# auggiemarignier/pxmcmc

Measured on AMD Instinct MI355X. Metric: MYULA samples/sec at L=256 synthesis, higher is better.
Workload: dtype f64

## Files before the change

### include/pxmcmc_amd.h

```cpp
#ifndef PXMCMC_AMD_H
#define PXMCMC_AMD_H

#include <stddef.h>
#include <stdint.h>

#ifdef __cplusplus
extern "C" {
#endif

typedef struct pxm_sht_plan_s* pxm_sht_plan_t;
typedef struct pxm_wav_plan_s* pxm_wav_plan_t;
typedef struct pxm_dwav_plan_s* pxm_dwav_plan_t;
typedef struct pxm_hwav_plan_s* pxm_hwav_plan_t;
typedef void* pxm_stream_t;

int pxm_version(void);
#ifdef PXM_NOISE_F64
#error "the -DPXM_NOISE_F64 build switch was removed: pass the flag PXM_NOISE_F64 per call (one library serves both precisions)"
#endif
#define PXM_NOISE_F64 16
int pxm_noise_bits(void);
int64_t pxm_host_check_address_ranges(int L, double B, int J_min, int spin, int max_chains, int what);
const char* pxm_last_error(void);
int pxm_device_count(void);
// ... 74 lines not shown

#define PXM_MODE_REAL_NOISE 0
#define PXM_MODE_CPLX_NOISE 1
#define PXM_MODE_REAL_PAIRS 2
int pxm_wav_gradg_step(pxm_wav_plan_t plan, const void* X, const void* preds, const void* data,
                       const void* invcov, int invcov_complex, const double* T, double T_scalar,
                       double delta, double lmda, const void* noise, int mode,
                       uint64_t seed, uint64_t chain0, uint64_t iter, void* X_out, int C,
                       pxm_stream_t stream);

int pxm_wav_image_init(pxm_wav_plan_t plan, const void* preds, const void* data, const void* invcov,
                       int invcov_complex, int C, pxm_stream_t stream);
int pxm_wav_image_step(pxm_wav_plan_t plan, const void* X, const void* data, const void* invcov,
                       int invcov_complex, const double* T, double T_scalar, double delta, double lmda,
                       const void* noise, int mode, uint64_t seed, uint64_t chain0, uint64_t iter,
                       void* X_out, void* preds_out, int C, pxm_stream_t stream);

int pxm_wav_ring_set_data(pxm_wav_plan_t plan, const void* data, pxm_stream_t stream);
int pxm_wav_ring_init(pxm_wav_plan_t plan, const void* X, int C, pxm_stream_t stream);
int pxm_wav_ring_step(pxm_wav_plan_t plan, const void* X, double w_re, double w_im, const double* T,
                      double T_scalar, double delta, double lmda, const void* noise, int mode,
                      uint64_t seed, uint64_t chain0, uint64_t iter, void* X_out, int C, pxm_stream_t stream);
int pxm_wav_ring_preds(pxm_wav_plan_t plan, void* preds, int C, pxm_stream_t stream);

int pxm_wav_wl_attach(pxm_wav_plan_t plan, const int32_t* pix2data, const double* weight, int64_t ndata);
int pxm_wav_wl_uses_recursion(pxm_wav_plan_t plan);
int pxm_wav_wl_forward(pxm_wav_plan_t plan, const void* X, void* gamma, int C, pxm_stream_t stream);
int pxm_wav_wl_adjoint(pxm_wav_plan_t plan, const void* gamma, const void* data, const void* invcov,
                       int invcov_complex, void* X_out, int C, pxm_stream_t stream);

int pxm_soft(const void* X, const double* T, double T_scalar, void* out, int64_t n, int C, int dtype,
             pxm_stream_t stream);
int pxm_residual_grad(const void* preds, const void* data, const void* invcov, int invcov_complex,
                      void* out, int64_t n, int C, int dtype, pxm_stream_t stream);
int pxm_myula_step(const void* X, const void* gradg, const double* T, double T_scalar,
                   const double* delta_dev, double delta, double lmda, const void* noise,
                   int noise_complex, uint64_t seed, uint64_t chain0, uint64_t iter,
                   const uint64_t* iter_dev, void* X_out, int64_t n, int C, int dtype,
                   pxm_stream_t stream);
int pxm_chain_step(const void* X, const void* proxf, const void* gradg, const double* delta_dev,
                   double delta, double lmda, const void* noise, int noise_complex, uint64_t seed,
                   uint64_t chain0, uint64_t iter, const uint64_t* iter_dev, void* X_out, int64_t n,
                   int C, int dtype, pxm_stream_t stream);
int pxm_skrock_stage(const void* U, const void* proxf, const double* T, double T_scalar, const void* gradg,
                     const void* V, double a, double b, double c, double e, double r, const void* noise,
                     int noise_complex, uint64_t seed, uint64_t chain0, uint64_t iter, const uint64_t* iter_dev,
// ... 53 lines not shown
```

### pxmcmc_amd/_lib.py

```python
import ctypes as C
import os

import torch

_HERE = os.path.dirname(os.path.abspath(__file__))
LIB_PATH = os.environ.get("PXM_LIB_PATH") or os.path.join(_HERE, "lib", "libpxmcmc_amd.so")

c_i64, c_u64, c_int, c_dbl, c_vp = C.c_int64, C.c_uint64, C.c_int, C.c_double, C.c_void_p

SIGNATURES = {
    "pxm_version": (c_int, []),
    "pxm_noise_bits": (c_int, []),
    "pxm_host_check_address_ranges": (c_i64, [c_int, c_dbl, c_int, c_int, c_int, c_int]),
    "pxm_last_error": (C.c_char_p, []),
    "pxm_device_count": (c_int, []),
    "pxm_capture_begin": (c_int, []),
    "pxm_capture_end": (c_int, []),
    "pxm_deferred_pending": (c_int, []),
    "pxm_tables_trim": (c_int, []),
    "pxm_wav_set_iter_counter": (c_int, [c_vp, c_vp]),
    "pxm_wav_release_iter_counter": (c_int, [c_vp, c_vp]),
    "pxm_wav_iter_counter_add": (c_int, [c_vp, c_u64, c_vp]),
    "pxm_wav_exact_dft_scales": (c_int, [c_vp]),
    "pxm_wav_status": (c_int, [c_vp, c_int, c_vp]),
    "pxm_sht_status": (c_int, [c_vp, c_int, c_vp]),
    "pxm_wav_profile_enable": (c_int, [c_vp, c_int]),
    "pxm_wav_profile_read": (c_int, [c_vp, c_vp, c_vp, c_vp, c_vp]),
    "pxm_wav_profile_read_launches": (c_int, [c_vp, c_vp, c_vp, c_vp, c_i64, c_vp]),
    "pxm_wav_profile_read_dft": (c_int, [c_vp, c_vp, c_vp, c_vp]),
    "pxm_wav_workspace_nonfinite": (c_i64, [c_vp, c_vp]),
    "pxm_reduce_scratch_doubles": (c_i64, [c_int]),
    "pxm_j_max": (c_int, [c_int, c_dbl]),
    "pxm_wav_bandlimits": (c_int, [c_int, c_dbl, c_int, c_vp, c_int]),
    "pxm_wav_ncoefs": (c_i64, [c_int, c_dbl, c_int, c_vp]),
    "pxm_tiling_axisym": (c_int, [c_int, c_dbl, c_int, c_vp, c_vp]),
    "pxm_mw_ring_weights": (c_int, [c_int, c_vp]),
# ... 146 lines not shown
```

### pxmcmc_amd/csrc/plans.hip

```cpp
#include "../../include/pxmcmc_amd.h"
#include "elem.h"
#include "sht_core.h"
#include "sht_rec.h"

#include <algorithm>
#include <cmath>
#include <cstdlib>
#include <cstring>
#include <map>
#include <string>
#include <memory>
#include <mutex>

namespace pxm {

struct TaskList {
  GemmTask* d = nullptr;
  int n = 0;
  bool paired = false;
  int nslab = 2;
  std::vector<int> bls;
  std::vector<int> los;
  double mfma_units = 0;
  bool gram = false;
  double gram_table_bytes = 0;
  int flags = 0;
  int pk = 0;
  std::vector<char> tab_shared;
};

static int upload_tasks(std::vector<GemmTask> v, bool paired, TaskList* out, std::vector<int> bls, int ncol,
                        const double* ws_base, const char* name, std::vector<int> los = {}, int pk = 0,
                        std::vector<char> tab_shared = {}) {
  out->pk = pk;
  tab_shared.resize(bls.size(), 0);
  out->tab_shared = tab_shared;
  out->bls = bls;
  los.resize(bls.size(), 0);
  out->los = los;
  const char* order_env = getenv("PXM_GEMM_ORDER");
  const std::string order = order_env ? order_env : (v.size() > 2048 ? "xcd" : "bins");
  const int64_t fixed = order == "xcd" ? 32 : 0;
  auto work = [fixed](const GemmTask& a) { return (int64_t)(a.k_end - a.k_beg + fixed) * a.n_rt; };
  std::stable_sort(v.begin(), v.end(), [&](const GemmTask& a, const GemmTask& b) { return work(a) > work(b); });
  if (order == "xcd" && !v.empty()) {
    constexpr int NQ = 8;
    std::map<int64_t, int> unit_of;
    std::vector<std::vector<GemmTask>> units;
    for (const GemmTask& t : v) {
      auto it = unit_of.find(t.x_off[0]);
// ... 57 lines not shown
    }
    v.swap(ordered);
  }
  out->n = (int)v.size();
  out->paired = paired;
  out->nslab = pk ? 4 : (paired ? 2 : 1);
  for (const GemmTask& t : v) {
    PXM_REQUIRE(t.n_rt >= 0 && t.n_rt <= 8 && t.row0 >= 0 && t.row0 % 16 == 0 && t.k_beg >= 0 && t.k_beg % 16 == 0 &&
                    (t.n_rt == 0 || (t.k_end > t.k_beg && (t.k_end - t.k_beg) % 16 == 0)),
                "upload_tasks: malformed GEMM task");
    out->mfma_units += (double)t.n_rt * ((t.k_end - t.k_beg) / 4) * (pk ? 1 : t.nslab);
    for (int sl = 0; sl < 4; ++sl)
      if (t.x2_off[sl]) out->flags |= 1;
    if (t.ks_off[0] || t.ks_off[1]) out->flags |= 2;
  }
  if (v.empty()) return 0;
  if (int rc = check_gemm_task_ranges(v, out->nslab, out->flags, ncol, ws_base, name)) return rc;
  if (int rc = dev_alloc(&out->d, v.size() * sizeof(GemmTask), "GEMM task list")) return rc;
  return dev_upload(out->d, v.data(), v.size() * sizeof(GemmTask));
}

static double tasklist_bytes(const TaskList& tl, int cg) {
  double bytes = 0;
  for (size_t i = 0; i < tl.bls.size(); ++i) {
    const double Ld = tl.bls[i];
    if (tl.gram) bytes += tl.gram_table_bytes + 3 * 16.0 * cg * Ld * Ld + 16.0 * Ld * Ld;
    else bytes += gemm_alg_bytes(tl.bls[i], tl.paired, cg, tl.los[i]);
    if (!tl.gram && tl.pk && tl.tab_shared[i]) bytes -= gemm_table_bytes(tl.bls[i], tl.paired, tl.los[i]);
  }
  return bytes;
}

static int run_tasks(const TaskList& tl, const double* X, double* Y, int ncol, int C, hipStream_t st,
                     const GemmAffine& aff = GemmAffine(), Profiler* prof = nullptr) {
  note_stream(st);
  if (tl.pk)
    return launch_gemm_packed(tl.d, tl.n, tl.pk, tl.flags, X, Y, ncol, 0, tasklist_bytes(tl, C), tl.mfma_units * 2048.0, st, prof);
  for (int col0 = 0; col0 < ncol; col0 += 32) {
    const int ct = (ncol - col0 >= 32) ? 2 : 1;
    const int cg = std::max(0, std::min(C - col0 / 2, 8 * ct));
    if (cg == 0) break;
    const double bytes = tasklist_bytes(tl, cg);
    GemmAffine a = aff;
    if (col0) a.bump = nullptr;
    a.ncol_live = 2 * C;
    int rc = launch_gemm(tl.d, tl.n, tl.nslab, tl.flags, X, Y, ncol, col0, ct, bytes, tl.mfma_units * ct * 2048.0, st, a, prof);
// ... 213 lines not shown
  *out = &sp;
  return 0;
}
}

struct pxm_wav_plan_s {
  int L = 0, J_min = 0, J_max = 0, Cmax = 0, Cp = 0, ncol = 0, Rp = 0;
  int spin = 0;
  double B = 0;
  int nsc = 0;
  std::vector<int> bl;
  std::vector<int64_t> coef_off;
  int64_t ncoefs = 0;
  std::vector<ShtTables*> T;
  ShtTables* TL = nullptr;
  std::vector<DftPlan> dft;
  DftPlan dftL;
  double* ws = nullptr;
  std::vector<int64_t> offG;
  int64_t offGL = 0, offHL = 0, offS = 0;
  int64_t offGD = 0, offHD = 0;
  int64_t offHDc = 0;
  TaskList gram, adj_invadj_D;
  bool have_data_rings = false;
  int64_t offHA = 0, offHB = 0;
  double* d_kc_syn = nullptr;
  double* d_kc_ana = nullptr;
  TaskList syn_fwd, syn_inv, adj_invadj, adj_fwdadj;
  TaskList ana_fwd, ana_inv, anadj_invadj, anadj_fwdadj;
  int64_t table_bytes[2] = {0, 0};
  static constexpr int NSIDE = 3;
  static constexpr int nside = 2;
  hipStream_t side[NSIDE] = {nullptr, nullptr, nullptr};
  hipEvent_t ev_fork = nullptr, ev_join[NSIDE] = {nullptr, nullptr, nullptr};
  bool plain_group = true;
  std::vector<int> lane_of;
  DftGroupList dft_group;
  int pk = 0;
  int twin_s = -1;
  bool wl_failed = false;
  double* d_twin = nullptr;
  int64_t offGT = 0;
  int ncol_t = 0;
  double* d_g2n = nullptr;
  int ncol_g2 = 0;
  double* d_hn = nullptr;
// ... 136 lines not shown
    wav_hold(p, p->T[s]);
    rc = make_dft_plan(p->bl[s], &p->dft[s]);
    if (rc) return rc;
    p->dft[s].d_status = p->d_status;
  }
  rc = get_tables(L, spin, 0xF, &p->TL);
  if (rc) return rc;
  wav_hold(p, p->TL);
  rc = make_dft_plan(L, &p->dftL);
  if (rc) return rc;
  p->dftL.d_status = p->d_status;
  int64_t w = 0;
  p->offGL = w; w += arr_size(L, p->ncol);
  p->offHL = w; w += arr_size(L, p->ncol);
  p->offGD = w; w += arr_size(L, p->ncol);
  p->offHD = w; w += arr_size(L, p->ncol);
  p->offHDc = w; w += (int64_t)(2 * L - 1) * p->Rp * 2;
  p->offHA = w; w += arr_size(L, p->ncol);
  p->offHB = w; w += arr_size(L, p->ncol);
  p->plain_group = !getenv("PXM_NO_PLAIN_DFT_GROUP");
  for (int s = 0; s < p->nsc; ++s) {
    p->offG.push_back(w); w += arr_size(p->bl[s], p->ncol);
  }
  p->offG2 = w; w += arr_size(L, p->ncol);
  p->offS = w; w += (int64_t)p->Rp * p->ncol;
  if ((rc = dev_alloc(&p->ws, (size_t)w * sizeof(double), "wavelet plan workspace"))) return rc;
  if ((rc = dev_zero(p->ws, (size_t)w * sizeof(double)))) return rc;
  std::vector<double> k0, kap;
  tiling_axisym(L, B, J_min, k0, kap);
  std::vector<double> kc_syn((size_t)p->nsc * p->Rp, 0.0), kc_ana((size_t)p->nsc * p->Rp, 0.0);
  const double cs = std::sqrt(2.0 * M_PI), ca = 1.0 / std::sqrt(2.0 * M_PI);
  for (int s = 0; s < p->nsc; ++s)
    for (int el = std::abs(spin); el < p->bl[s]; ++el) {
      const double k = (s == 0) ? k0[el] : kap[(size_t)(J_min + s - 1) * L + el];
      kc_syn[(size_t)s * p->Rp + el] = (s == 0) ? k : cs * k;
      kc_ana[(size_t)s * p->Rp + el] = (s == 0) ? k : ca * k;
    }
  if ((rc = dev_alloc(&p->d_kc_syn, kc_syn.size() * sizeof(double), "synthesis kernel rows c kappa [nsc][Rp]"))) return rc;
  if ((rc = dev_alloc(&p->d_kc_ana, kc_ana.size() * sizeof(double), "analysis kernel rows c kappa [nsc][Rp]"))) return rc;
  if ((rc = dev_upload(p->d_kc_syn, kc_syn.data(), kc_syn.size() * sizeof(double)))) return rc;
  if ((rc = dev_upload(p->d_kc_ana, kc_ana.data(), kc_ana.size() * sizeof(double)))) return rc;
  std::vector<int> el_lo(p->nsc, 0);
  for (int s = 0; s < p->nsc; ++s)
    while (el_lo[s] < p->bl[s] && kc_syn[(size_t)s * p->Rp + el_lo[s]] == 0.0) ++el_lo[s];
  std::vector<GemmTask> v_syn_fwd, v_adj_fwdadj, v_ana_inv, v_anadj_invadj, v;
  p->el_lo_s = el_lo;
// ... 60 lines not shown

extern "C" {

int pxm_wav_plan_create(int L, double B, int J_min, int max_chains, unsigned flags, pxm_wav_plan_t* plan) {
  (void)flags;
  return wav_plan_create_impl("pxm_wav_plan_create", L, B, J_min, 0, max_chains, plan);
}

int pxm_wav_plan_create_spin(int L, double B, int J_min, int spin, int max_chains, unsigned flags, pxm_wav_plan_t* plan) {
  (void)flags;
  return wav_plan_create_impl("pxm_wav_plan_create_spin", L, B, J_min, spin, max_chains, plan);
}

int pxm_wav_plan_destroy(pxm_wav_plan_t p) {
  if (!p) return 0;
  dft_group_destroy(&p->dft_group);
  for (auto& d : p->dft) free_dft_plan(&d);
  free_dft_plan(&p->dftL);
  deferred_free(p->ws);
  deferred_free(p->d_kc_syn);
  deferred_free(p->d_kc_ana);
  deferred_free(p->d_wlk);
  deferred_free(p->d_status);
  TaskList* tls[] = {&p->syn_fwd, &p->syn_inv, &p->adj_invadj, &p->adj_fwdadj, &p->gram, &p->adj_invadj_D,
                     &p->ana_fwd, &p->ana_inv, &p->anadj_invadj, &p->anadj_fwdadj, &p->wl_inv, &p->wl_invadj};
  for (TaskList* t : tls) free_tasks(t);
  profiler_release(&p->prof);
  for (ShtTables* T : p->held) release_tables(T);
  rec_tables_destroy(p->rec2);
  deferred_free(p->d_twin);
  deferred_free(p->d_g2n);
  deferred_free(p->d_hn);
  deferred_free(p->d_gn);
  dft_group_destroy(&p->dft_group_n);
  free_tasks(&p->wl_syn_fwd);
  free_tasks(&p->wl_adj_fwdadj);
  delete p;
  drain_deferred();
  return 0;
}

int pxm_wav_set_iter_counter(pxm_wav_plan_t p, uint64_t* counter_dev) {
  PXM_REQUIRE(p, "pxm_wav_set_iter_counter: null plan");
  PXM_REQUIRE(!counter_dev || !p->iter_dev || p->iter_dev == counter_dev,
              "pxm_wav_set_iter_counter: this plan already has a live iteration counter (one stepping engine per plan "
              "at a time; release the first with pxm_wav_release_iter_counter)");
  p->iter_dev = counter_dev;
// ... 329 lines not shown
    if ((rc = wav_rings_update_rings(p, out, C, st))) return rc;
  } else {
    if ((rc = wav_rings_to_blocks(p, out, C, st))) return rc;
    if ((rc = wav_blocks_to_rings(p, X_out, C, st))) return rc;
  }
  if ((rc = run_tasks(p->syn_fwd, p->ws, p->ws, p->ncol, C, st, GemmAffine(), &p->prof))) return rc;
  if ((rc = run_tasks(p->syn_inv, p->ws, p->ws, p->ncol, C, st, GemmAffine(), &p->prof))) return rc;
  PxOut po;
  po.f = (double*)preds_out;
  po.chain_stride = (int64_t)p->L * (2 * p->L - 1);
  if (dft_can_fuse(p->dftL)) {
    image_residual(po, data, invcov, invcov_complex);
    return launch_ring2px2ring(p->dftL, p->ws + p->offGL, p->ncol, po, C, st);
  }
  if ((rc = launch_ring2px(p->dftL, p->ws + p->offGL, p->ncol, po, C, st))) return rc;
  return pxm_wav_image_init(p, preds_out, data, invcov, invcov_complex, C, stream);
}

}
namespace pxm {
__global__ void k_pack_data_term(const double2* __restrict__ HD, double2* __restrict__ HDc, int64_t rows, int Cp) {
  for (int64_t i = blockIdx.x * (int64_t)blockDim.x + threadIdx.x; i < rows; i += (int64_t)gridDim.x * blockDim.x) HDc[i] = HD[i * Cp];
}
}
extern "C" {

static int wav_make_gram_lists(pxm_wav_plan_t p) {
  int rc;
  if (!p->gram.d) {
    if ((rc = get_tables(p->L, p->spin, 1u << TAB_GRAM, &p->TL))) return rc;
    wav_hold(p, p->TL);
    std::vector<GemmTask> v;
    GemmFuse fz;
    fz.x2_base = p->offHB;
    fz.hd_base = p->offHDc;
    fz.hd_stride = 2;
    append_gemm_tasks(*p->TL, TAB_GRAM, p->ncol, p->offHA, p->L, p->Rp, p->offHL, p->L, p->Rp, nullptr, p->offS, p->ws, v, 0, fz);
    if ((rc = upload_tasks(v, p->TL->paired, &p->gram, {p->L}, p->ncol, p->ws, "Gram step"))) return rc;
    p->gram.gram = true;
    p->gram.gram_table_bytes = (double)p->TL->bytes[TAB_GRAM];
    v.clear();
    append_gemm_tasks(*p->TL, TAB_INV_ADJ, p->ncol, p->offGD, p->L, p->Rp, p->offHD, p->L, p->Rp, nullptr, p->offS, p->ws, v);
    if ((rc = upload_tasks(v, p->TL->paired, &p->adj_invadj_D, {p->L}, p->ncol, p->ws, "inverse-adjoint of the data rings"))) return rc;
  }
  return 0;
}

int pxm_wav_ring_set_data(pxm_wav_plan_t p, const void* data, pxm_stream_t stream) {
  PXM_REQUIRE(p && data, "pxm_wav_ring_set_data: null argument");
  hipStream_t st = (hipStream_t)stream;
  int rc;
  if ((rc = wav_make_gram_lists(p))) return rc;
  PxIn in;
  in.f = (const double*)data;
  in.chain_stride = (int64_t)p->L * (2 * p->L - 1);
  if ((rc = launch_px2ring(p->dftL, in, p->ws + p->offGD, p->ncol, 1, st))) return rc;
  if ((rc = run_tasks(p->adj_invadj_D, p->ws, p->ws, p->ncol, 1, st, GemmAffine(), &p->prof))) return rc;
  const int64_t rows = (int64_t)(2 * p->L - 1) * p->Rp;
  hipLaunchKernelGGL(k_pack_data_term, dim3((unsigned)std::min<int64_t>((rows + 255) / 256, 2048)), dim3(256), 0, st,
                     reinterpret_cast<const double2*>(p->ws + p->offHD), reinterpret_cast<double2*>(p->ws + p->offHDc), rows,
                     p->ncol / 2);
  PXM_HIP(hipGetLastError());
  p->have_data_rings = true;
  return 0;
}

static int wav_coeffs_to_rings(pxm_wav_plan_t p, const void* X, int C, hipStream_t st, uint64_t* bump = nullptr) {
  int rc;
  if ((rc = wav_blocks_to_rings(p, X, C, st, bump))) return rc;
  return run_tasks(p->syn_fwd, p->ws, p->ws, p->ncol, C, st, GemmAffine(), &p->prof);
}

int pxm_wav_ring_init(pxm_wav_plan_t p, const void* X, int C, pxm_stream_t stream) {
  int rc = wav_check(p, X, X, C, "pxm_wav_ring_init");
  return rc ? rc : wav_coeffs_to_rings(p, X, C, (hipStream_t)stream);
}

int pxm_wav_ring_preds(pxm_wav_plan_t p, void* preds, int C, pxm_stream_t stream) {
  int rc = wav_check(p, preds, preds, C, "pxm_wav_ring_preds");
// ... 1 lines not shown
  hipStream_t st = (hipStream_t)stream;
  if ((rc = run_tasks(p->syn_inv, p->ws, p->ws, p->ncol, C, st, GemmAffine(), &p->prof))) return rc;
  PxOut out;
  out.f = (double*)preds;
  out.chain_stride = (int64_t)p->L * (2 * p->L - 1);
  return launch_ring2px(p->dftL, p->ws + p->offGL, p->ncol, out, C, st);
}

int pxm_wav_ring_step(pxm_wav_plan_t p, const void* X, double w_re, double w_im, const double* T, double T_scalar,
                      double delta, double lmda, const void* noise, int mode, uint64_t seed, uint64_t chain0,
                      uint64_t iter, void* X_out, int C, pxm_stream_t stream) {
  int rc = wav_check(p, X, X_out, C, "pxm_wav_ring_step");
  if (rc) return rc;
  PXM_REQUIRE(p->have_data_rings, "pxm_wav_ring_step: call pxm_wav_ring_set_data first");
  PxOut out;
  if ((rc = wav_update_out(p, "pxm_wav_ring_step", X, T, T_scalar, delta, lmda, noise, mode, seed, chain0, iter, X_out, &out))) return rc;
  hipStream_t st = (hipStream_t)stream;
  GemmAffine aff;
  aff.on = 1;
  aff.ns = (double)(2 * p->L - 1);
  aff.wr = w_re;
  aff.wi = w_im;
  aff.bump = p->iter_dev;
  if ((rc = run_tasks(p->gram, p->ws, p->ws, p->ncol, C, st, aff, &p->prof))) return rc;
  if ((rc = run_tasks(p->adj_fwdadj, p->ws, p->ws, p->ncol, C, st, GemmAffine(), &p->prof))) return rc;
  if (wav_can_fuse_dft(p)) {
    if ((rc = wav_rings_update_rings(p, out, C, st))) return rc;
    if ((rc = run_tasks(p->syn_fwd, p->ws, p->ws, p->ncol, C, st, GemmAffine(), &p->prof))) return rc;
    return 0;
  }
  if ((rc = wav_rings_to_blocks(p, out, C, st))) return rc;
  return wav_coeffs_to_rings(p, X_out, C, st);
}

static int wl_attach_impl(pxm_wav_plan_t p, const int32_t* pix2data, const double* weight, int64_t ndata) {
  PXM_REQUIRE(p->L >= 3, "pxm_wav_wl_attach: Bandlimit must be at least 3 for a spin-2 field");
  const int64_t P = (int64_t)p->L * (2 * p->L - 1);
  PXM_REQUIRE(ndata >= 0 && ndata <= P && (pix2data || ndata == P), "pxm_wav_wl_attach: bad mask description");
  int rc;
  if (!p->T2 && !p->rec2) {
    std::vector<double> k((size_t)p->Rp, 0.0);
    for (int el = 2; el < p->L; ++el) k[el] = -std::sqrt(((el + 2.0) * (el - 1.0)) / ((el + 1.0) * el));
    if ((rc = dev_alloc(&p->d_wlk, k.size() * sizeof(double), "weak-lensing harmonic kernel k_l [Rp]"))) return rc;
    if ((rc = dev_upload(p->d_wlk, k.data(), k.size() * sizeof(double)))) return rc;
  }
  int twin_cand = -1;
  if (p->twin_s < 0 && p->pk == 2 && p->Cmax == 1)
    for (int s = 0; s + 1 < p->nsc && twin_cand < 0; ++s)
      if (p->bl[s + 1] == p->bl[s] && p->T[s + 1] == p->T[s] && !wav_in_group(p, s) && !wav_in_group(p, s + 1)) twin_cand = s;
  if (!p->T2 && !p->rec2 && rec_wanted(p->L, 2, p->Cmax)) {
    p->ncol_g2 = 2 * p->Cmax;
    if (p->ncol_g2 != p->ncol) {
      const size_t nb = (size_t)(2 * p->L - 1) * p->Rp * p->ncol_g2 * sizeof(double);
      if ((rc = dev_alloc(&p->d_g2n, nb, "narrow spin-2 ring array"))) return rc;
      if ((rc = dev_zero(p->d_g2n, nb))) return rc;
// ... 173 lines not shown
  std::lock_guard<std::mutex> lock(mu);
  PXM_REQUIRE(!capture_in_progress(), "pxm_host_check_address_ranges: not during a stream capture");
  set_dry_run(true);
  ranges_checked_reset();
  int rc = 0;
  if (what & 1) {
    pxm_sht_plan_t sp = nullptr;
    rc = pxm_sht_plan_create(L, spin, max_chains, 0, &sp);
    if (sp) pxm_sht_plan_destroy(sp);
  }
  if (!rc && (what & 2)) {
    pxm_wav_plan_t wp = nullptr;
    const int wspin = (what & 8) ? spin : 0;
    rc = pxm_wav_plan_create_spin(L, B, J_min, wspin, max_chains, 0, &wp);
    if (!rc) rc = wav_make_gram_lists(wp);
    if (!rc && (what & 4) && L >= 3 && wspin == 0) rc = pxm_wav_wl_attach(wp, nullptr, nullptr, (int64_t)L * (2 * L - 1));
    if (wp) pxm_wav_plan_destroy(wp);
  }
  tables_trim();
  set_dry_run(false);
  return rc ? -1 : ranges_checked();
}

}
```

### pxmcmc_amd/csrc/sht_core.h

```cpp
#pragma once
#include "common.h"

namespace pxm {

enum TableKind { TAB_INV = 0, TAB_FWD = 1, TAB_INV_ADJ = 2, TAB_FWD_ADJ = 3, TAB_GRAM = 4, TAB_KINDS = 5 };
inline bool kind_el_to_ring(int kind) { return kind == TAB_INV || kind == TAB_FWD_ADJ; }
inline bool kind_rows_are_el(int kind) { return kind == TAB_FWD || kind == TAB_INV_ADJ || kind == TAB_GRAM; }
inline bool kind_k_is_el(int kind) { return kind == TAB_INV || kind == TAB_FWD_ADJ || kind == TAB_GRAM; }

struct GemmTask {
  int64_t tab_off;
  int64_t rt_stride;
  int64_t x_off[4];
  int64_t y_off[4];
  int64_t x2_off[4];
  int64_t hd_off[4];
  int64_t ks_off[2];
  int64_t rs_off[2];
  int row_lo[2], row_hi[2];
  int k_beg, k_end;
  int row0;
  int n_rt;
  int nslab;
  double sign1;
// ... 41 lines not shown
  int64_t x2_base = -1;
  const double* rscale = nullptr;
  int row_lo = 0, row_hi = 1 << 30;
  int64_t hd_base = -1;
  int hd_stride = 0;
};

struct ShtTables {
  int L = 0, spin = 0, Rp = 0;
  bool paired = false;
  int n_m = 0;
  double* d_tab[TAB_KINDS] = {nullptr, nullptr, nullptr, nullptr, nullptr};
  size_t bytes[TAB_KINDS] = {0, 0, 0, 0, 0};
  std::vector<int64_t> m_off[TAB_KINDS];
  std::vector<int> k_beg[TAB_KINDS];
  int refs = 0;
  int m_of(int i) const { return paired ? i : i - (L - 1); }
};

int get_tables(int L, int spin, unsigned kinds_mask, ShtTables** out);
void retain_tables(ShtTables* T);
void release_tables(ShtTables* T);
int64_t tables_trim();

void append_gemm_tasks(const ShtTables& T, int kind, int ncol, int64_t x_base, int x_L, int x_Rp,
                       int64_t y_base, int y_L, int y_Rp, const double* kscale, int64_t scratch_off,
                       const double* ws_base, std::vector<GemmTask>& tasks, int el_lo = 0,
                       const GemmFuse& fuse = GemmFuse());
struct GemmSide {
  int64_t x_base, y_base;
  int x_L, x_Rp, y_L, y_Rp;
  const double* kscale;
  int el_lo;
  GemmFuse fuse;
  int x_ncol = 0, y_ncol = 0;
};

void append_gemm_tasks_packed(const ShtTables& T, int kind, int ncol, const GemmSide& side_a, const GemmSide* side_b,
                              int64_t scratch_off, const double* ws_base, std::vector<GemmTask>& tasks);
int launch_gemm_packed(const GemmTask* d_tasks, int n_tasks, int pk, int flags, const double* X, double* Y, int ncol, int col0,
                       double alg_bytes, double flops, hipStream_t stream, Profiler* prof = nullptr);

int launch_gemm(const GemmTask* d_tasks, int n_tasks, int nslab, int flags, const double* X, double* Y, int ncol,
                int col0, int ct, double alg_bytes, double flops, hipStream_t stream,
                const GemmAffine& aff = GemmAffine(), Profiler* prof = nullptr);

inline double gemm_table_bytes(int L, bool paired, int el_lo = 0) {
  double tab_entries = 0;
  for (int m = paired ? 0 : -(L - 1); m < L; ++m) {
    const int am = m < 0 ? -m : m;
    const int n = L - (am > el_lo ? am : el_lo);
    if (n > 0) tab_entries += n;
  }
  return 8.0 * L * tab_entries;
}
inline double gemm_alg_bytes(int L, bool paired, int C, int el_lo = 0) {
  double tab_entries = 0, lm_entries = 0;
  for (int m = paired ? 0 : -(L - 1); m < L; ++m) {
    const int am = m < 0 ? -m : m;
    const int n = L - (am > el_lo ? am : el_lo);
    if (n > 0) tab_entries += n;
  }
// ... 100 lines not shown
```

### pxmcmc_amd/csrc/sht_gemm.hip

```cpp
#include "../../include/pxmcmc_amd.h"
#include "sht_core.h"

#include <type_traits>

#include <hip/hip_ext.h>

#include <cstdlib>
#include <map>
#include <mutex>

namespace pxm {

typedef double d4 __attribute__((ext_vector_type(4)));

constexpr int KC = 16;
#define PXM_GEMM_MFMA(ACC, A, B) ACC = __builtin_amdgcn_mfma_f64_16x16x4f64(A, B, ACC, 0, 0, 0);
#ifdef PXM_GEMM_TRACE
__device__ unsigned long long* g_gemm_trace = nullptr;
extern "C" int pxm_debug_set_gemm_trace(unsigned long long* buf) {
  return hipMemcpyToSymbol(HIP_SYMBOL(g_gemm_trace), &buf, sizeof(buf)) == hipSuccess ? 0 : -1;
}
#endif
__device__ __forceinline__ double stage_add(double a, double b, bool on) { return a + (on ? b : 0.0); }
__device__ __forceinline__ double2 stage_add(double2 a, double2 b, bool on) { return double2{a.x + (on ? b.x : 0.0), a.y + (on ? b.y : 0.0)}; }
__device__ __forceinline__ double stage_scale(double a, double sc) { return a * sc; }
__device__ __forceinline__ double2 stage_scale(double2 a, double sc) { return double2{a.x * sc, a.y * sc}; }
template <int CT, int NSLAB>
struct GemmGeom {
  static constexpr int NCT = CT * NSLAB;
  static constexpr int COLS = 16 * NCT;
  static constexpr int PITCH = COLS + (COLS == 16 ? 0 : 16);
};
// ... 486 lines not shown
  const size_t first = tasks.size();
  append_tasks_impl(T, kind, ncol, sa, scratch_off, ws_base, tasks);
  for (size_t i = first; i < tasks.size(); ++i) {
    GemmTask& g = tasks[i];
    const int m = T.paired ? g.m_unit : g.m_unit - (T.L - 1);
    fill_side(g, 0, T, kind, m, ncol, side_a, scratch_off, ws_base);
    fill_side(g, 1, T, kind, m, ncol, side_b ? *side_b : side_a, scratch_off, ws_base);
    g.nslab = side_b ? 4 : 2;
    g.x_ncol = side_a.x_ncol ? side_a.x_ncol : ncol;
    g.y_ncol = side_a.y_ncol ? side_a.y_ncol : ncol;
    if (!T.paired) {
      g.nslab = 1;
    }
  }
}

void append_gemm_tasks(const ShtTables& T, int kind, int ncol, int64_t x_base, int x_L, int x_Rp,
                       int64_t y_base, int y_L, int y_Rp, const double* kscale, int64_t scratch_off,
                       const double* ws_base, std::vector<GemmTask>& tasks, int el_lo, const GemmFuse& fuse) {
  const GemmSide sd{x_base, y_base, x_L, x_Rp, y_L, y_Rp, kscale, el_lo, fuse};
  append_tasks_impl(T, kind, ncol, sd, scratch_off, ws_base, tasks);
}

__global__ void k_build_fwd(const double* __restrict__ Bd, const double* __restrict__ Qd, double* __restrict__ Ad,
                            int Rp, int L, double scale, int m0, int spin) {
  const int i = blockIdx.z;
  const int el = blockIdx.x * 16 + threadIdx.x, t = blockIdx.y * 16 + threadIdx.y;
  const int m = m0 + i;
  const int par = ((m + spin) & 1) ? 1 : 0;
  const double* B = Bd + (int64_t)i * Rp * Rp;
  const double* Q = Qd + (int64_t)par * Rp * Rp;
  double acc = 0;
  for (int tp = 0; tp < L; ++tp) acc += B[(int64_t)tp * Rp + el] * Q[(int64_t)tp * Rp + t];
  Ad[(int64_t)i * Rp * Rp + (int64_t)el * Rp + t] = scale * acc;
}

__global__ void k_build_gram(const double* __restrict__ Bd, double* __restrict__ Gd, int Rp, int L) {
  const int i = blockIdx.z;
  const int r = blockIdx.x * 16 + threadIdx.x, c = blockIdx.y * 16 + threadIdx.y;
  const double* B = Bd + (int64_t)i * Rp * Rp;
  double acc = 0;
  for (int t = 0; t < L; ++t) acc += B[(int64_t)t * Rp + r] * B[(int64_t)t * Rp + c];
  Gd[(int64_t)i * Rp * Rp + (int64_t)r * Rp + c] = acc;
}

__global__ void k_tile_table(const double* __restrict__ D, double* __restrict__ out, int Rp, int row_beg,
// ... 99 lines not shown
      PXM_HIP(hipGetLastError());
    }
    if (missing & (1u << TAB_GRAM)) {
      PXM_HIP(hipMalloc(&d_G, dense * sizeof(double)));
      dim3 grid(Rp / 16, Rp / 16, T->n_m), block(16, 16);
      hipLaunchKernelGGL(k_build_gram, grid, block, 0, 0, d_B, d_G, Rp, L);
      PXM_HIP(hipGetLastError());
    }
    for (int k = 0; k < TAB_KINDS; ++k)
      if (missing >> k & 1u) {
        int rc = build_kind(*T, k, d_B, d_A, d_G);
        if (rc) return rc;
      }
    PXM_HIP(hipDeviceSynchronize());
    PXM_HIP(hipFree(d_B));
    if (d_A) PXM_HIP(hipFree(d_A));
    if (d_Q) PXM_HIP(hipFree(d_Q));
    if (d_G) PXM_HIP(hipFree(d_G));
  }
  *out = T;
  return 0;
}

void retain_tables(ShtTables* T) {
  std::lock_guard<std::mutex> lock(g_tab_mutex);
  if (T) ++T->refs;
}
void release_tables(ShtTables* T) {
  std::lock_guard<std::mutex> lock(g_tab_mutex);
  if (T && T->refs > 0) --T->refs;
}
int64_t tables_trim() {
  std::lock_guard<std::mutex> lock(g_tab_mutex);
  int64_t freed = 0;
  for (auto it = g_tab_cache.begin(); it != g_tab_cache.end();) {
    ShtTables* T = it->second;
    if (T->refs > 0 || (dry_run() && it->first.first % 16 != 15)) {
      ++it;
      continue;
    }
    for (int k = 0; k < TAB_KINDS; ++k) {
      if (T->d_tab[k]) deferred_free(T->d_tab[k]);
      freed += (int64_t)T->bytes[k];
    }
    delete T;
    it = g_tab_cache.erase(it);
  }
  drain_deferred();
  return freed;
}

}
```

Before: 116,200.

## Fold Gram and forward-adjoint ring tables into one precomputed per-scale operator

For non-packed wavelet plans, the Gram matrix at L is precomputed together with each scale's forward-adjoint table and kernel weights into one folded table per scale and m. The ring step then runs a single GEMM task list per iteration instead of a Gram GEMM at full L followed by the forward-adjoint GEMM. The constant data term is pre-projected and packed per scale and fused into the folded GEMM. This removes the intermediate L-sized ring and a whole GEMM pass, at the cost of extra table memory, a one-time build kernel, and new debug and units entry points.

```diff
diff --git a/include/pxmcmc_amd.h b/include/pxmcmc_amd.h
--- a/include/pxmcmc_amd.h
+++ b/include/pxmcmc_amd.h
@@ -120,6 +120,8 @@
                       double T_scalar, double delta, double lmda, const void* noise, int mode,
                       uint64_t seed, uint64_t chain0, uint64_t iter, void* X_out, int C, pxm_stream_t stream);
 int pxm_wav_ring_preds(pxm_wav_plan_t plan, void* preds, int C, pxm_stream_t stream);
+int pxm_wav_ring_table_dense(pxm_wav_plan_t plan, int which, int s, int m, double* out);
+int pxm_host_wav_mfma_units(int L, double B, int J_min, int max_chains, double* forward_units, double* folded_units);
 
 int pxm_wav_wl_attach(pxm_wav_plan_t plan, const int32_t* pix2data, const double* weight, int64_t ndata);
 int pxm_wav_wl_uses_recursion(pxm_wav_plan_t plan);
diff --git a/pxmcmc_amd/_lib.py b/pxmcmc_amd/_lib.py
--- a/pxmcmc_amd/_lib.py
+++ b/pxmcmc_amd/_lib.py
@@ -12,6 +12,8 @@
     "pxm_version": (c_int, []),
     "pxm_noise_bits": (c_int, []),
     "pxm_host_check_address_ranges": (c_i64, [c_int, c_dbl, c_int, c_int, c_int, c_int]),
+    "pxm_host_wav_mfma_units": (c_int, [c_int, c_dbl, c_int, c_int, c_vp, c_vp]),
+    "pxm_wav_ring_table_dense": (c_int, [c_vp, c_int, c_int, c_int, c_vp]),
     "pxm_last_error": (C.c_char_p, []),
     "pxm_device_count": (c_int, []),
     "pxm_capture_begin": (c_int, []),
diff --git a/pxmcmc_amd/csrc/plans.hip b/pxmcmc_amd/csrc/plans.hip
--- a/pxmcmc_amd/csrc/plans.hip
+++ b/pxmcmc_amd/csrc/plans.hip
@@ -26,6 +26,9 @@
   double gram_table_bytes = 0;
   int flags = 0;
   int pk = 0;
+  bool fold = false;
+  double fold_table_bytes = 0;
+  int fold_L = 0;
   std::vector<char> tab_shared;
 };
 
@@ -129,6 +132,11 @@
 
 static double tasklist_bytes(const TaskList& tl, int cg) {
   double bytes = 0;
+  if (tl.fold) {
+    bytes = tl.fold_table_bytes + 2 * 16.0 * cg * tl.fold_L * tl.fold_L;
+    for (int b : tl.bls) bytes += 16.0 * (cg + 1) * b * (2.0 * b - 1);
+    return bytes;
+  }
   for (size_t i = 0; i < tl.bls.size(); ++i) {
     const double Ld = tl.bls[i];
     if (tl.gram) bytes += tl.gram_table_bytes + 3 * 16.0 * cg * Ld * Ld + 16.0 * Ld * Ld;
@@ -388,6 +396,9 @@
   int64_t offGD = 0, offHD = 0;
   int64_t offHDc = 0;
   TaskList gram, adj_invadj_D;
+  FoldTables* fold = nullptr;
+  TaskList adj_fold;
+  std::vector<int64_t> offC;
   bool have_data_rings = false;
   int64_t offHA = 0, offHB = 0;
   double* d_kc_syn = nullptr;
@@ -570,6 +581,9 @@
   for (int s = 0; s < p->nsc; ++s) {
     p->offG.push_back(w); w += arr_size(p->bl[s], p->ncol);
   }
+  for (int s = 0; s < p->nsc; ++s) {
+    p->offC.push_back(w); w += (int64_t)(2 * p->bl[s] - 1) * round_up(p->bl[s], 16) * 2;
+  }
   p->offG2 = w; w += arr_size(L, p->ncol);
   p->offS = w; w += (int64_t)p->Rp * p->ncol;
   if ((rc = dev_alloc(&p->ws, (size_t)w * sizeof(double), "wavelet plan workspace"))) return rc;
@@ -676,7 +690,8 @@
   deferred_free(p->d_kc_ana);
   deferred_free(p->d_wlk);
   deferred_free(p->d_status);
-  TaskList* tls[] = {&p->syn_fwd, &p->syn_inv, &p->adj_invadj, &p->adj_fwdadj, &p->gram, &p->adj_invadj_D,
+  release_fold_tables(p->fold);
+  TaskList* tls[] = {&p->syn_fwd, &p->syn_inv, &p->adj_invadj, &p->adj_fwdadj, &p->gram, &p->adj_fold, &p->adj_invadj_D,
                      &p->ana_fwd, &p->ana_inv, &p->anadj_invadj, &p->anadj_fwdadj, &p->wl_inv, &p->wl_invadj};
   for (TaskList* t : tls) free_tasks(t);
   profiler_release(&p->prof);
@@ -1052,12 +1067,47 @@
 __global__ void k_pack_data_term(const double2* __restrict__ HD, double2* __restrict__ HDc, int64_t rows, int Cp) {
   for (int64_t i = blockIdx.x * (int64_t)blockDim.x + threadIdx.x; i < rows; i += (int64_t)gridDim.x * blockDim.x) HDc[i] = HD[i * Cp];
 }
+__global__ void k_pack_const_rings(const double2* __restrict__ G, double2* __restrict__ Cs, int bl, int Rb, int Cp, int signed_) {
+  const int64_t rows = (int64_t)(2 * bl - 1) * Rb;
+  for (int64_t i = blockIdx.x * (int64_t)blockDim.x + threadIdx.x; i < rows; i += (int64_t)gridDim.x * blockDim.x) {
+    const int m = (int)(i / Rb) - (bl - 1);
+    const double sg = (signed_ && m < 0 && (m & 1)) ? -1.0 : 1.0;
+    const double2 v = G[i * Cp];
+    Cs[i] = double2{sg * v.x, sg * v.y};
+  }
+}
 }
 extern "C" {
+
+static bool wav_folds(const pxm_wav_plan_s* p) { return p->pk == 0; }
 
 static int wav_make_gram_lists(pxm_wav_plan_t p) {
   int rc;
-  if (!p->gram.d) {
+  if (wav_folds(p) && !p->adj_fold.d) {
+    if ((rc = get_tables(p->L, p->spin, 1u << TAB_GRAM, &p->TL))) return rc;
+    wav_hold(p, p->TL);
+    if ((rc = get_fold_tables(*p->TL, p->T, p->bl, p->d_kc_syn, p->B, p->J_min, &p->fold))) return rc;
+    retain_fold_tables(p->fold);
+    drop_table_kind(p->TL, TAB_GRAM);
+    std::vector<GemmTask> v;
+    for (int s = 0; s < p->nsc; ++s) {
+      GemmSide g = wav_side(p, s, 1);
+      g.x_base = p->offHA;
+      g.fuse.x2_base = p->offHB;
+      g.kscale = nullptr;
+      g.fuse.hd_base = p->offC[s];
+      g.fuse.hd_stride = 2;
+      append_fold_tasks(*p->fold, s, *p->TL, p->ncol, g, p->offS, p->ws, v);
+    }
+    if ((rc = upload_tasks(v, p->TL->paired, &p->adj_fold, p->bl, p->ncol, p->ws, "folded Gram + forward-adjoint (all scales)"))) return rc;
+    p->adj_fold.fold = true;
+    p->adj_fold.fold_table_bytes = (double)p->fold->bytes;
+    p->adj_fold.fold_L = p->L;
+    v.clear();
+    append_gemm_tasks(*p->TL, TAB_INV_ADJ, p->ncol, p->offGD, p->L, p->Rp, p->offHL, p->L, p->Rp, nullptr, p->offS, p->ws, v);
+    if ((rc = upload_tasks(v, p->TL->paired, &p->adj_invadj_D, {p->L}, p->ncol, p->ws, "inverse-adjoint of the data rings"))) return rc;
+  }
+  if (!wav_folds(p) && !p->gram.d) {
     if ((rc = get_tables(p->L, p->spin, 1u << TAB_GRAM, &p->TL))) return rc;
     wav_hold(p, p->TL);
     std::vector<GemmTask> v;
@@ -1085,6 +1135,20 @@
   in.f = (const double*)data;
   in.chain_stride = (int64_t)p->L * (2 * p->L - 1);
   if ((rc = launch_px2ring(p->dftL, in, p->ws + p->offGD, p->ncol, 1, st))) return rc;
+  if (wav_folds(p)) {
+    if ((rc = run_tasks(p->adj_invadj_D, p->ws, p->ws, p->ncol, 1, st, GemmAffine(), &p->prof))) return rc;
+    if ((rc = run_tasks(p->adj_fwdadj, p->ws, p->ws, p->ncol, 1, st, GemmAffine(), &p->prof))) return rc;
+    for (int s = 0; s < p->nsc; ++s) {
+      const int b = p->bl[s], Rb = round_up(b, 16);
+      const int64_t rows = (int64_t)(2 * b - 1) * Rb;
+      hipLaunchKernelGGL(k_pack_const_rings, dim3((unsigned)std::min<int64_t>((rows + 255) / 256, 2048)), dim3(256), 0, st,
+                         reinterpret_cast<const double2*>(p->ws + p->offG[s]), reinterpret_cast<double2*>(p->ws + p->offC[s]), b,
+                         Rb, p->ncol / 2, p->fold->paired ? 1 : 0);
+    }
+    PXM_HIP(hipGetLastError());
+    p->have_data_rings = true;
+    return 0;
+  }
   if ((rc = run_tasks(p->adj_invadj_D, p->ws, p->ws, p->ncol, 1, st, GemmAffine(), &p->prof))) return rc;
   const int64_t rows = (int64_t)(2 * p->L - 1) * p->Rp;
   hipLaunchKernelGGL(k_pack_data_term, dim3((unsigned)std::min<int64_t>((rows + 255) / 256, 2048)), dim3(256), 0, st,
@@ -1132,8 +1196,12 @@
   aff.wr = w_re;
   aff.wi = w_im;
   aff.bump = p->iter_dev;
-  if ((rc = run_tasks(p->gram, p->ws, p->ws, p->ncol, C, st, aff, &p->prof))) return rc;
-  if ((rc = run_tasks(p->adj_fwdadj, p->ws, p->ws, p->ncol, C, st, GemmAffine(), &p->prof))) return rc;
+  if (wav_folds(p)) {
+    if ((rc = run_tasks(p->adj_fold, p->ws, p->ws, p->ncol, C, st, aff, &p->prof))) return rc;
+  } else {
+    if ((rc = run_tasks(p->gram, p->ws, p->ws, p->ncol, C, st, aff, &p->prof))) return rc;
+    if ((rc = run_tasks(p->adj_fwdadj, p->ws, p->ws, p->ncol, C, st, GemmAffine(), &p->prof))) return rc;
+  }
   if (wav_can_fuse_dft(p)) {
     if ((rc = wav_rings_update_rings(p, out, C, st))) return rc;
     if ((rc = run_tasks(p->syn_fwd, p->ws, p->ws, p->ncol, C, st, GemmAffine(), &p->prof))) return rc;
@@ -1141,6 +1209,16 @@
   }
   if ((rc = wav_rings_to_blocks(p, out, C, st))) return rc;
   return wav_coeffs_to_rings(p, X_out, C, st);
+}
+
+int pxm_wav_ring_table_dense(pxm_wav_plan_t p, int which, int s, int m, double* out) {
+  PXM_REQUIRE(p && out && which >= 0 && which <= 2, "pxm_wav_ring_table_dense: bad arguments");
+  PXM_REQUIRE(p->fold, "pxm_wav_ring_table_dense: the plan has no folded tables (few-chain plan, or no pxm_wav_ring_set_data yet)");
+  PXM_REQUIRE(which == 2 || (s >= 0 && s < p->nsc), "pxm_wav_ring_table_dense: no such scale");
+  if (which == 0) return untile_table(p->fold, s, nullptr, 0, m, out);
+  if (which == 1) return untile_table(nullptr, 0, p->T[s], TAB_FWD_ADJ, m, out);
+  if (int rc = get_tables(p->L, p->spin, 1u << TAB_GRAM, &p->TL)) return rc;
+  return untile_table(nullptr, 0, p->TL, TAB_GRAM, m, out);
 }
 
 static int wl_attach_impl(pxm_wav_plan_t p, const int32_t* pix2data, const double* weight, int64_t ndata) {
@@ -1360,4 +1438,21 @@
   return rc ? -1 : ranges_checked();
 }
 
-}
+int pxm_host_wav_mfma_units(int L, double B, int J_min, int max_chains, double* forward_units, double* folded_units) {
+  PXM_REQUIRE(forward_units && folded_units, "pxm_host_wav_mfma_units: null output");
+  PXM_REQUIRE(!capture_in_progress(), "pxm_host_wav_mfma_units: not during a stream capture");
+  set_dry_run(true);
+  pxm_wav_plan_t wp = nullptr;
+  int rc = pxm_wav_plan_create(L, B, J_min, max_chains, 0, &wp);
+  if (!rc) rc = wav_make_gram_lists(wp);
+  if (!rc) {
+    *forward_units = wp->syn_fwd.mfma_units;
+    *folded_units = wp->adj_fold.mfma_units;
+  }
+  if (wp) pxm_wav_plan_destroy(wp);
+  tables_trim();
+  set_dry_run(false);
+  return rc;
+}
+
+}
diff --git a/pxmcmc_amd/csrc/sht_core.h b/pxmcmc_amd/csrc/sht_core.h
--- a/pxmcmc_amd/csrc/sht_core.h
+++ b/pxmcmc_amd/csrc/sht_core.h
@@ -1,5 +1,8 @@
 #pragma once
 #include "common.h"
+
+#include <algorithm>
+#include <cstdlib>
 
 namespace pxm {
 
@@ -87,6 +90,24 @@
 void retain_tables(ShtTables* T);
 void release_tables(ShtTables* T);
 int64_t tables_trim();
+void drop_table_kind(ShtTables* T, int kind);
+
+struct FoldTables {
+  int L = 0, Rp = 0, J_min = 0, spin = 0;
+  bool paired = true;
+  int k_beg(int m) const { return round_down(std::max(std::abs(m), std::abs(spin)), 16); }
+  double B = 0;
+  double* d = nullptr;
+  size_t bytes = 0;
+  std::vector<int> bl;
+  std::vector<std::vector<int64_t>> m_off;
+  int refs = 0;
+};
+int get_fold_tables(const ShtTables& TL, const std::vector<ShtTables*>& Ts, const std::vector<int>& bl, const double* d_kc,
+                    double B, int J_min, FoldTables** out);
+void retain_fold_tables(FoldTables* F);
+void release_fold_tables(FoldTables* F);
+int untile_table(const FoldTables* F, int s, const ShtTables* T, int kind, int m, double* out_host);
 
 void append_gemm_tasks(const ShtTables& T, int kind, int ncol, int64_t x_base, int x_L, int x_Rp,
                        int64_t y_base, int y_L, int y_Rp, const double* kscale, int64_t scratch_off,
@@ -103,6 +124,8 @@
 
 void append_gemm_tasks_packed(const ShtTables& T, int kind, int ncol, const GemmSide& side_a, const GemmSide* side_b,
                               int64_t scratch_off, const double* ws_base, std::vector<GemmTask>& tasks);
+void append_fold_tasks(const FoldTables& F, int s, const ShtTables& TL, int ncol, const GemmSide& side, int64_t scratch_off,
+                       const double* ws_base, std::vector<GemmTask>& tasks);
 int launch_gemm_packed(const GemmTask* d_tasks, int n_tasks, int pk, int flags, const double* X, double* Y, int ncol, int col0,
                        double alg_bytes, double flops, hipStream_t stream, Profiler* prof = nullptr);
 
diff --git a/pxmcmc_amd/csrc/sht_gemm.hip b/pxmcmc_amd/csrc/sht_gemm.hip
--- a/pxmcmc_amd/csrc/sht_gemm.hip
+++ b/pxmcmc_amd/csrc/sht_gemm.hip
@@ -7,7 +7,9 @@
 
 #include <cstdlib>
 #include <map>
+#include <memory>
 #include <mutex>
+#include <tuple>
 
 namespace pxm {
 
@@ -540,6 +542,34 @@
   append_tasks_impl(T, kind, ncol, sd, scratch_off, ws_base, tasks);
 }
 
+void append_fold_tasks(const FoldTables& F, int s, const ShtTables& TLs, int ncol, const GemmSide& side, int64_t scratch_off,
+                       const double* ws_base, std::vector<GemmTask>& tasks) {
+  const int b = F.bl[s], Rb = round_up(b, 16);
+  const int rpt = gemm_rows_per_task(ncol);
+  for (int i = 0; i < (int)F.m_off[s].size(); ++i) {
+    const int m = F.paired ? i : i - (b - 1);
+    const int kb = F.k_beg(m);
+    if (kb >= F.Rp) continue;
+    const int64_t rt_stride = (int64_t)((F.Rp - kb) / 8) * 128;
+    const int n_rt_total = Rb / 16;
+    for (int rt = 0; rt < n_rt_total; rt += rpt) {
+      GemmTask g;
+      g.m_unit = F.paired ? m : m + F.L - 1;
+      g.tab_off = (F.d + F.m_off[s][i] + (int64_t)rt * rt_stride) - ws_base;
+      g.rt_stride = rt_stride;
+      for (int grp = 0; grp < 2; ++grp) fill_side(g, grp, TLs, TAB_FWD_ADJ, m, ncol, side, scratch_off, ws_base);
+      g.nslab = F.paired ? 2 : 1;
+      g.k_beg = kb;
+      g.k_end = F.Rp;
+      g.row0 = 16 * rt;
+      g.n_rt = std::min(rpt, n_rt_total - rt);
+      g.sign1 = (m & 1) ? -1.0 : 1.0;
+      g.x_ncol = g.y_ncol = ncol;
+      tasks.push_back(g);
+    }
+  }
+}
+
 __global__ void k_build_fwd(const double* __restrict__ Bd, const double* __restrict__ Qd, double* __restrict__ Ad,
                             int Rp, int L, double scale, int m0, int spin) {
   const int i = blockIdx.z;
@@ -685,6 +715,163 @@
   return 0;
 }
 
+void drop_table_kind(ShtTables* T, int kind) {
+  std::lock_guard<std::mutex> lock(g_tab_mutex);
+  if (!T || T->refs > 1 || !T->d_tab[kind]) return;
+  deferred_free(T->d_tab[kind]);
+  T->d_tab[kind] = nullptr;
+  T->bytes[kind] = 0;
+}
+
+__device__ __forceinline__ int64_t tiled_index(int row, int k, int row_beg, int k_beg, int nk2) {
+  const int r = row - row_beg, c = k - k_beg;
+  return ((int64_t)(r >> 4) * nk2 + (c >> 3)) * 128 + ((r & 15) + 16 * (c & 3)) * 2 + ((c >> 2) & 1);
+}
+__global__ void k_build_fold(const double* __restrict__ FA, const int64_t* __restrict__ fa_off, const double* __restrict__ G,
+                             const int64_t* __restrict__ g_off, const double* __restrict__ kc, double* __restrict__ out,
+                             const int64_t* __restrict__ out_off, int Rb, int Rp, int m0, int spin) {
+  const int i = blockIdx.z, m = m0 + i, am = m < 0 ? -m : m, as = spin < 0 ? -spin : spin;
+  const int kba = am & ~15, kb = (am > as ? am : as) & ~15;
+  const int nk2 = (Rp - kb) / 8, nk2a = (Rb - kba) / 8;
+  const int kk2 = blockIdx.x, rt = blockIdx.y;
+  if (kk2 >= nk2) return;
+  const int lane = threadIdx.x >> 1, h = threadIdx.x & 1;
+  const int t = 16 * rt + (lane & 15);
+  const int lp = kb + 8 * kk2 + 4 * h + (lane >> 4);
+  const double* fa = FA + fa_off[i];
+  const double* g = G + g_off[i];
+  double acc = 0;
+  for (int l = kb; l < Rb; ++l) {
+    const double k = kc[l];
+    if (k != 0.0) acc += fa[tiled_index(t, l, 0, kba, nk2a)] * k * g[tiled_index(l, lp, kb, kb, nk2)];
+  }
+  out[out_off[i] + ((int64_t)rt * nk2 + kk2) * 128 + threadIdx.x] = (m < 0 && (m & 1)) ? -acc : acc;
+}
+__global__ void k_untile_table(const double* __restrict__ tiled, double* __restrict__ dense, int ncols, int row_beg, int k_beg,
+                               int nk2) {
+  const int rt = blockIdx.y, kk2 = blockIdx.x;
+  const int lane = threadIdx.x >> 1, h = threadIdx.x & 1;
+  const int row = row_beg + 16 * rt + (lane & 15), k = k_beg + 8 * kk2 + 4 * h + (lane >> 4);
+  dense[(int64_t)row * ncols + k] = tiled[((int64_t)rt * nk2 + kk2) * 128 + threadIdx.x];
+}
+
+struct FoldKey {
+  int L, J_min, spin, dev;
+  double B;
+  bool operator<(const FoldKey& o) const { return std::tie(L, J_min, spin, dev, B) < std::tie(o.L, o.J_min, o.spin, o.dev, o.B); }
+};
+static std::map<FoldKey, FoldTables*> g_fold_cache;
+
+int get_fold_tables(const ShtTables& TL, const std::vector<ShtTables*>& Ts, const std::vector<int>& bl, const double* d_kc,
+                    double B, int J_min, FoldTables** out) {
+  std::lock_guard<std::mutex> lock(g_tab_mutex);
+  PXM_REQUIRE(TL.d_tab[TAB_GRAM], "get_fold_tables: needs the Gram table at L");
+  int dev = 15;
+  if (!dry_run()) PXM_HIP(hipGetDevice(&dev));
+  const FoldKey key{TL.L, J_min, TL.spin, dev, B};
+  auto it = g_fold_cache.find(key);
+  if (it != g_fold_cache.end()) {
+    *out = it->second;
+    return 0;
+  }
+  std::unique_ptr<FoldTables> F(new FoldTables());
+  F->L = TL.L;
+  F->Rp = TL.Rp;
+  F->B = B;
+  F->J_min = J_min;
+  F->spin = TL.spin;
+  F->paired = TL.paired;
+  F->bl = bl;
+  const int Rp = TL.Rp, nsc = (int)bl.size();
+  int64_t total = 0;
+  F->m_off.resize(nsc);
+  for (int s = 0; s < nsc; ++s) {
+    const int Rb = round_up(bl[s], 16);
+    PXM_REQUIRE(Ts[s] && Ts[s]->paired && Ts[s]->L == bl[s] && Ts[s]->Rp == Rb && Ts[s]->d_tab[TAB_FWD_ADJ] && Rb <= Rp,
+                "get_fold_tables: scale tables do not match the plan");
+    for (int m = F->paired ? 0 : -(bl[s] - 1); m < bl[s]; ++m) {
+      F->m_off[s].push_back(total);
+      total += (int64_t)(Rb / 16) * ((Rp - F->k_beg(m)) / 8) * 128;
+    }
+  }
+  F->bytes = (size_t)total * sizeof(double);
+  if (int rc = dev_alloc(&F->d, F->bytes, "folded Gram x forward-adjoint ring tables")) return rc;
+  if (!dry_run()) {
+    for (int s = 0; s < nsc; ++s) {
+      const int b = bl[s], Rb = round_up(b, 16);
+      const int n = (int)F->m_off[s].size(), m0 = F->paired ? 0 : -(b - 1);
+      std::vector<int64_t> off((size_t)3 * n);
+      for (int i = 0; i < n; ++i) {
+        const int m = m0 + i, am = std::abs(m), ig = F->paired ? m : m + TL.L - 1;
+        off[i] = Ts[s]->m_off[TAB_FWD_ADJ][am];
+        off[n + i] = TL.m_off[TAB_GRAM][ig];
+        off[2 * n + i] = F->m_off[s][i];
+        PXM_REQUIRE(Ts[s]->k_beg[TAB_FWD_ADJ][am] == round_down(am, 16) && TL.k_beg[TAB_GRAM][ig] == F->k_beg(m),
+                    "get_fold_tables: unexpected table start");
+      }
+      int64_t* d_off = nullptr;
+      PXM_HIP(hipMalloc(&d_off, off.size() * sizeof(int64_t)));
+      PXM_HIP(hipMemcpy(d_off, off.data(), off.size() * sizeof(int64_t), hipMemcpyHostToDevice));
+      dim3 grid(Rp / 8, Rb / 16, n), block(128);
+      hipLaunchKernelGGL(k_build_fold, grid, block, 0, 0, Ts[s]->d_tab[TAB_FWD_ADJ], d_off, TL.d_tab[TAB_GRAM], d_off + n,
+                         d_kc + (size_t)s * Rp, F->d, d_off + 2 * n, Rb, Rp, m0, F->spin);
+      const hipError_t e = hipGetLastError();
+      const hipError_t e2 = hipDeviceSynchronize();
+      (void)hipFree(d_off);
+      if (e != hipSuccess || e2 != hipSuccess) {
+        deferred_free(F->d);
+        PXM_HIP(e != hipSuccess ? e : e2);
+      }
+    }
+  }
+  *out = g_fold_cache[key] = F.release();
+  return 0;
+}
+void retain_fold_tables(FoldTables* F) {
+  std::lock_guard<std::mutex> lock(g_tab_mutex);
+  if (F) ++F->refs;
+}
+void release_fold_tables(FoldTables* F) {
+  std::lock_guard<std::mutex> lock(g_tab_mutex);
+  if (F && F->refs > 0) --F->refs;
+}
+
+int untile_table(const FoldTables* F, int s, const ShtTables* T, int kind, int m, double* out_host) {
+  std::lock_guard<std::mutex> lock(g_tab_mutex);
+  const double* src;
+  int nrows, ncols, row_beg, k_beg;
+  if (F) {
+    PXM_REQUIRE(s >= 0 && s < (int)F->bl.size() && std::abs(m) < F->bl[s] && (m >= 0 || !F->paired),
+                "untile_table: no such folded table");
+    src = F->d + F->m_off[s][F->paired ? m : m + F->bl[s] - 1];
+    nrows = round_up(F->bl[s], 16);
+    ncols = F->Rp;
+    row_beg = 0;
+    k_beg = F->k_beg(m);
+  } else {
+    PXM_REQUIRE(T && (kind == TAB_FWD_ADJ || kind == TAB_GRAM) && T->d_tab[kind] && std::abs(m) < T->L && (m >= 0 || !T->paired),
+                "untile_table: no such table");
+    const int i = T->paired ? m : m + T->L - 1;
+    src = T->d_tab[kind] + T->m_off[kind][i];
+    nrows = ncols = T->Rp;
+    k_beg = T->k_beg[kind][i];
+    row_beg = kind_rows_are_el(kind) ? k_beg : 0;
+  }
+  const size_t nb = (size_t)nrows * ncols * sizeof(double);
+  double* d = nullptr;
+  PXM_HIP(hipMalloc(&d, nb));
+  hipError_t e = hipMemset(d, 0, nb);
+  dim3 grid((ncols - k_beg) / 8, (nrows - row_beg) / 16), block(128);
+  if (e == hipSuccess && grid.x && grid.y) {
+    hipLaunchKernelGGL(k_untile_table, grid, block, 0, 0, src, d, ncols, row_beg, k_beg, (ncols - k_beg) / 8);
+    e = hipGetLastError();
+  }
+  if (e == hipSuccess) e = hipMemcpy(out_host, d, nb, hipMemcpyDeviceToHost);
+  (void)hipFree(d);
+  PXM_HIP(e);
+  return 0;
+}
+
 void retain_tables(ShtTables* T) {
   std::lock_guard<std::mutex> lock(g_tab_mutex);
   if (T) ++T->refs;
@@ -709,6 +896,17 @@
     delete T;
     it = g_tab_cache.erase(it);
   }
+  for (auto it = g_fold_cache.begin(); it != g_fold_cache.end();) {
+    FoldTables* F = it->second;
+    if (F->refs > 0 || (dry_run() && it->first.dev != 15)) {
+      ++it;
+      continue;
+    }
+    deferred_free(F->d);
+    freed += (int64_t)F->bytes;
+    delete F;
+    it = g_fold_cache.erase(it);
+  }
   drain_deferred();
   return freed;
 }
```

After: 111,600. 0.96x the previous value.
